# orybkin/video-gcp

Measured on AMD Instinct MI355X. Metric: predicted frames/sec, 64x64x3 seq_len=80 gcp_tree (posterior forward + all loss terms, model(inputs) and model.loss() of train.py:157-159, batch-stat BatchNorm), higher is better.
Workload: dtype f32 (encoder / decoder convs and the tree GEMMs from 512 rows: split-f16 MFMA with f32 accumulate, f32-equivalent; everything else exact f32 MFMA)

## Files before the change

video-gcp_amd/csrc/conv_enc_split.hip:

```cpp
#include "common.h"

#include <cstdlib>

namespace {

typedef _Float16 h8 __attribute__((ext_vector_type(8)));

__device__ __forceinline__ f32x4 mfma32h(h8 a, h8 b, f32x4 c) {
    return __builtin_amdgcn_mfma_f32_16x16x32_f16(a, b, c, 0, 0, 0);
}

template <int CIN, int COUT, int HIN, int FPB, int WP, int WC, bool ZP>
struct EncSplitCfg {
    static constexpr int HOUT = HIN / 2, CT = COUT / 16, CTW = CT / WC;
    static constexpr int PIXB = CIN * 4 + 16;
    static constexpr int NG = FPB * HOUT * HOUT / 16, PGW = (NG + WP - 1) / WP;
    static constexpr int FRAME_PIX = HIN * HIN;
    static constexpr int NSTEP = CIN == 16 ? 8 : 16 * (CIN / 32);
    static constexpr int lds_bytes(int fpb) { return fpb * FRAME_PIX * PIXB + (ZP ? PIXB : 0); }
    static constexpr int LDS_BYTES = lds_bytes(FPB);
    static_assert(WP * WC == 4 && CT % WC == 0 && (HOUT * HOUT) % 16 == 0 && (CIN == 16 || CIN % 32 == 0), "tiling");
};

template <int CIN, int COUT, int HIN, int FPB, int WP, int WC, bool ZP>
__global__ void __launch_bounds__(256) conv4x4s2_split_kernel(const gcpx_conv_args a, const int nblk, const int nrows, const int fpb) {
    using Cfg = EncSplitCfg<CIN, COUT, HIN, FPB, WP, WC, ZP>;
    constexpr int HOUT = Cfg::HOUT, CT = Cfg::CT, CTW = Cfg::CTW, PIXB = Cfg::PIXB, PGW = Cfg::PGW, NSTEP = Cfg::NSTEP;
    constexpr int FRAME_PIX = Cfg::FRAME_PIX, C4 = CIN / 4, C8 = CIN / 8;
    const int tot4 = fpb * FRAME_PIX * C4, tot8 = fpb * FRAME_PIX * C8;
    const int ngrp = fpb * HOUT * HOUT / 16;
    const int npg = __builtin_amdgcn_readfirstlane((ngrp - (int)((threadIdx.x >> 6) % WP) + WP - 1) / WP);
    extern __shared__ float4 encs_smem4[];
    char* lds = reinterpret_cast<char*>(encs_smem4);
    const int tid = threadIdx.x, lane = tid & 63, wave = tid >> 6;
    const int wp = wave % WP, wc = wave / WP;
    const int j = lane & 15, q = lane >> 4;
    const gcpx_conv_src s = a.src[0];
    const int zero_off = fpb * FRAME_PIX * PIXB;
    float* wmax = reinterpret_cast<float*>(lds + CIN * 4);
    if (ZP && tid < PIXB / 4) reinterpret_cast<float*>(lds + zero_off)[tid] = 0.f;
    float4 sc4 = make_float4(1.f, 1.f, 1.f, 1.f), sh4 = make_float4(0.f, 0.f, 0.f, 0.f);
    if (s.scale) {
        sc4 = *reinterpret_cast<const float4*>(s.scale + 4 * (tid % C4));
        sh4 = *reinterpret_cast<const float4*>(s.shift + 4 * (tid % C4));
    }
    const int ew = a.w_split_log2_dev ? __builtin_amdgcn_readfirstlane(*a.w_split_log2_dev) : a.w_split_log2;

    f32x4 st1[CTW], st2[CTW];
#pragma unroll
    for (int ct = 0; ct < CTW; ++ct) { st1[ct] = f32x4{0, 0, 0, 0}; st2[ct] = f32x4{0, 0, 0, 0}; }

    int base[PGW], fl_[PGW], pin_[PGW];
    unsigned vmask[PGW];
#pragma unroll
    for (int pt = 0; pt < PGW; ++pt) {
        const int p = (wp + pt * WP) * 16 + j;
        const int fl = p / (HOUT * HOUT), pin = p % (HOUT * HOUT);
        const int oy = pin / HOUT, ox = pin % HOUT;
        fl_[pt] = fl; pin_[pt] = pin;
        base[pt] = ((fl * HIN + 2 * oy - 1) * HIN + 2 * ox - 1) * PIXB;
        unsigned m = 0;
        for (int k = 0; k < 4; ++k) {
            if (2 * oy - 1 + k >= 0 && 2 * oy - 1 + k < HIN) m |= 1u << k;
            if (2 * ox - 1 + k >= 0 && 2 * ox - 1 + k < HIN) m |= 16u << k;
        }
        vmask[pt] = m;
    }
    const char* wbase = reinterpret_cast<const char*>(a.wpk_split) + (size_t)(wc * CTW) * 2048 + lane * 16;

    for (int blk = blockIdx.x; blk < nblk; blk += gridDim.x) {
        const int f0 = blk * fpb;
        __syncthreads();
        const float4* src = reinterpret_cast<const float4*>(s.ptr) + (size_t)f0 * FRAME_PIX * C4;
        const int nvalid4 = min(fpb, a.F - f0) * FRAME_PIX * C4;
        static_assert(256 % C4 == 0, "staging batches");
        float amax = 0.f;
#pragma unroll 1
        for (int i0 = 0; i0 < tot4; i0 += 256 * 8) {
            float4 v[8];
#pragma unroll
            for (int k = 0; k < 8; ++k) {
                const int idx = i0 + k * 256 + tid;
                v[k] = idx < nvalid4 ? src[idx] : make_float4(0.f, 0.f, 0.f, 0.f);
            }
#pragma unroll
            for (int k = 0; k < 8; ++k) {
                const int idx = i0 + k * 256 + tid;
                const int c4 = idx % C4, pix = idx / C4;
                if (idx < nvalid4) {
                    float4 x = v[k];
                    x.x = fmaf(x.x, sc4.x, sh4.x); x.y = fmaf(x.y, sc4.y, sh4.y); x.z = fmaf(x.z, sc4.z, sh4.z); x.w = fmaf(x.w, sc4.w, sh4.w);
                    if (s.act == GCPX_ACT_LRELU) { x.x = lrelu(x.x, 0.2f); x.y = lrelu(x.y, 0.2f); x.z = lrelu(x.z, 0.2f); x.w = lrelu(x.w, 0.2f); }
                    v[k] = x;
                    amax = fmaxf(amax, fmaxf(fmaxf(fabsf(x.x), fabsf(x.y)), fmaxf(fabsf(x.z), fabsf(x.w))));
                }
                if (idx < tot4) *reinterpret_cast<float4*>(lds + pix * PIXB + 16 * c4) = v[k];
            }
        }
#pragma unroll
        for (int m = 1; m < 64; m <<= 1) amax = fmaxf(amax, __shfl_xor(amax, m));
        if (lane == 0) wmax[wave] = amax;
        __syncthreads();
        amax = fmaxf(fmaxf(wmax[0], wmax[1]), fmaxf(wmax[2], wmax[3]));
        int ex = 14 + 127 - (int)((__float_as_uint(amax) >> 23) & 0xff);
        ex = __builtin_amdgcn_readfirstlane(amax > 0.f ? max(-100, min(min(100, 126 - ew), ex)) : min(100, 126 - ew));
        const float sx2 = __uint_as_float((unsigned)(127 + ex) << 23);
        for (int i = tid; i < tot8; i += 256) {
            const int c8 = i % C8, pix = i / C8;
            char* p = lds + pix * PIXB + 32 * c8;
            const float4 v0 = *reinterpret_cast<const float4*>(p), v1 = *reinterpret_cast<const float4*>(p + 16);
            const float f[8] = {v0.x * sx2, v0.y * sx2, v0.z * sx2, v0.w * sx2, v1.x * sx2, v1.y * sx2, v1.z * sx2, v1.w * sx2};
            h8 p1, p2;
#pragma unroll
            for (int e = 0; e < 8; ++e) {
                p1[e] = (_Float16)f[e];
                p2[e] = (_Float16)fmaf((float)p1[e], -1.f, f[e]);
            }
            *reinterpret_cast<h8*>(p) = p1;
            *reinterpret_cast<h8*>(p + 16) = p2;
        }
        __syncthreads();

        f32x4 acc[CTW][PGW];
#pragma unroll
        for (int ct = 0; ct < CTW; ++ct)
#pragma unroll
            for (int pt = 0; pt < PGW; ++pt) acc[ct][pt] = f32x4{0, 0, 0, 0};
        auto fetch_w = [&](const int step, h8 (&w)[CTW][2]) __attribute__((always_inline)) {
            const char* wp_ = wbase + (size_t)step * CT * 2048;
#pragma unroll
            for (int ct = 0; ct < CTW; ++ct) {
                w[ct][0] = *reinterpret_cast<const h8*>(wp_ + ct * 2048);
                w[ct][1] = *reinterpret_cast<const h8*>(wp_ + ct * 2048 + 1024);
            }
        };
        auto mm = [&](const int step, const h8 (&w)[CTW][2]) __attribute__((always_inline)) {
            const int tap = CIN == 16 ? 2 * step + (q >> 1) : CIN == 32 ? step : step >> 1;
            const int grp = CIN == 16 ? (q & 1) : CIN == 32 ? q : 4 * (step & 1) + q;
            const int ky = tap >> 2, kx = tap & 3;
            const int tapoff = (ky * HIN + kx) * PIXB + grp * 32;
            h8 b[PGW][2];
#pragma unroll
            for (int pt = 0; pt < PGW; ++pt) {
                if (pt >= npg) break;
                const bool ok = ((vmask[pt] >> ky) & 1u) && ((vmask[pt] >> (4 + kx)) & 1u);
                if constexpr (ZP) {
                    const char* p = lds + (ok ? base[pt] + tapoff : zero_off);
                    b[pt][0] = *reinterpret_cast<const h8*>(p);
                    b[pt][1] = *reinterpret_cast<const h8*>(p + 16);
                } else {
                    const char* p = lds + (ok ? base[pt] + tapoff : 0);
                    const h8 t0 = *reinterpret_cast<const h8*>(p), t1 = *reinterpret_cast<const h8*>(p + 16);
                    const h8 z = {0, 0, 0, 0, 0, 0, 0, 0};
                    b[pt][0] = ok ? t0 : z;
                    b[pt][1] = ok ? t1 : z;
                }
            }
#pragma unroll
            for (int ct = 0; ct < CTW; ++ct)
#pragma unroll
                for (int pt = 0; pt < PGW; ++pt) {
                    if (pt >= npg) break;
                    acc[ct][pt] = mfma32h(w[ct][1], b[pt][0], acc[ct][pt]);
                }
#pragma unroll
            for (int ct = 0; ct < CTW; ++ct)
#pragma unroll
                for (int pt = 0; pt < PGW; ++pt) {
                    if (pt >= npg) break;
                    acc[ct][pt] = mfma32h(w[ct][0], b[pt][1], acc[ct][pt]);
                }
#pragma unroll
            for (int ct = 0; ct < CTW; ++ct)
#pragma unroll
                for (int pt = 0; pt < PGW; ++pt) {
                    if (pt >= npg) break;
                    acc[ct][pt] = mfma32h(w[ct][0], b[pt][0], acc[ct][pt]);
                }
        };
        h8 wA[CTW][2], wB[CTW][2];
        static_assert(NSTEP % 2 == 0, "ping-pong");
        fetch_w(0, wA);
#pragma unroll 1
        for (int step = 0; step < NSTEP; step += 2) {
            fetch_w(step + 1, wB);
            mm(step, wA);
            fetch_w(step + 2 < NSTEP ? step + 2 : step, wA);
            mm(step + 1, wB);
        }
        const float inv = __uint_as_float((unsigned)(127 - ex - ew) << 23);
#pragma unroll
        for (int pt = 0; pt < PGW; ++pt) {
            const int f = f0 + fl_[pt];
            if (f >= a.F || wp + pt * WP >= ngrp) continue;
            float* op = a.out + ((size_t)f * HOUT * HOUT + pin_[pt]) * COUT;
#pragma unroll
            for (int ct = 0; ct < CTW; ++ct) {
                const int c = (wc * CTW + ct) * 16 + q * 4;
                const float4 bv = *reinterpret_cast<const float4*>(a.bias + c);
                f32x4 v = acc[ct][pt];
                v[0] = fmaf(v[0], inv, bv.x); v[1] = fmaf(v[1], inv, bv.y); v[2] = fmaf(v[2], inv, bv.z); v[3] = fmaf(v[3], inv, bv.w);
                if (a.out_act == GCPX_ACT_LRELU) {
                    v[0] = lrelu(v[0], 0.2f); v[1] = lrelu(v[1], 0.2f); v[2] = lrelu(v[2], 0.2f); v[3] = lrelu(v[3], 0.2f);
                }
                *reinterpret_cast<float4*>(op + c) = make_float4(v[0], v[1], v[2], v[3]);
                if (a.stats_partial) { st1[ct] += v; st2[ct] += v * v; }
            }
        }
    }
    if (a.stats_partial) {
        __syncthreads();
        float* red = reinterpret_cast<float*>(lds);
#pragma unroll
        for (int ct = 0; ct < CTW; ++ct) {
#pragma unroll
            for (int r = 0; r < 4; ++r) {
                const float s1 = row16_sum(st1[ct][r]);
                const float s2 = row16_sum(st2[ct][r]);
                if (j == 0) {
                    const int c = (wc * CTW + ct) * 16 + q * 4 + r;
                    red[(wp * 2 + 0) * CT * 16 + c] = s1;
                    red[(wp * 2 + 1) * CT * 16 + c] = s2;
                }
            }
        }
        __syncthreads();
        for (int i = tid; i < 2 * CT * 16; i += 256) {
            const int which = i / (CT * 16), c = i % (CT * 16);
            float sum = 0.f;
#pragma unroll
            for (int w_ = 0; w_ < WP; ++w_) sum += red[(w_ * 2 + which) * CT * 16 + c];
            a.stats_partial[((size_t)blockIdx.x * 2 + which) * CT * 16 + c] = sum;
            for (int r = blockIdx.x + gridDim.x; r < nrows; r += gridDim.x) a.stats_partial[((size_t)r * 2 + which) * CT * 16 + c] = 0.f;
        }
    }
}

template <int CIN, int COUT, int HIN, int FPB, int WP, int WC, bool ZP>
int launch_enc_split(const gcpx_conv_args* a, hipStream_t stream, int nrows, int cus) {
    using Cfg = EncSplitCfg<CIN, COUT, HIN, FPB, WP, WC, ZP>;
    auto kern = conv4x4s2_split_kernel<CIN, COUT, HIN, FPB, WP, WC, ZP>;
    static bool attr_set = false;
    if (!attr_set) {
        hipError_t e = hipFuncSetAttribute(reinterpret_cast<const void*>(kern), hipFuncAttributeMaxDynamicSharedMemorySize, Cfg::LDS_BYTES);
        if (e != hipSuccess) {
            gcpx_set_error("conv4x4s2 (split): hipFuncSetAttribute(%d B): %s", Cfg::LDS_BYTES, hipGetErrorString(e));
            return GCPX_ERR_HIP;
        }
        attr_set = true;
    }
    int fpb = 1;
    double best = -1.0;
    const double frame_bytes = 4.0 * (HIN * HIN * CIN + Cfg::HOUT * Cfg::HOUT * COUT);
    const double bank_bytes = 4.0 * 16 * CIN * COUT * (4 / WC) / WP;
    for (int c = 1; c <= FPB; ++c) {
        const int nb = (a->F + c - 1) / c;
        const double cost = (double)((nb + cus - 1) / cus) * (c * frame_bytes + bank_bytes);
        if (best < 0 || cost <= best) { best = cost; fpb = c; }
    }
    if (const char* e = getenv("GCPX_ENC_FPB")) { const int v = atoi(e); if (v >= 1 && v <= FPB) fpb = v; }
    const int nblk = (a->F + fpb - 1) / fpb;
    const int grid = nblk < nrows ? nblk : nrows;
    hipLaunchKernelGGL(kern, dim3(grid), dim3(256), Cfg::lds_bytes(fpb), stream, *a, nblk, nrows, fpb);
    return GCPX_OK;
}

}

int gcpx_launch_enc_split(const gcpx_conv_args* a, hipStream_t stream, int nrows, int cus) {
    if (a->Hin != a->Win) return 1;
    if (a->Cin == 16 && a->Cout == 32 && a->Hin == 32) return launch_enc_split<16, 32, 32, 1, 2, 2, false>(a, stream, nrows, cus);
    if (a->Cin == 32 && a->Cout == 64 && a->Hin == 16) return launch_enc_split<32, 64, 16, 4, 1, 4, true>(a, stream, nrows, cus);
    if (a->Cin == 64 && a->Cout == 128 && a->Hin == 8) return launch_enc_split<64, 128, 8, 8, 1, 4, true>(a, stream, nrows, cus);
    if (a->Cin == 16 && a->Cout == 32 && a->Hin == 16) return launch_enc_split<16, 32, 16, 4, 2, 2, true>(a, stream, nrows, cus);
    if (a->Cin == 32 && a->Cout == 64 && a->Hin == 8) return launch_enc_split<32, 64, 8, 16, 1, 4, true>(a, stream, nrows, cus);
    return 1;
}
```

Measured before the change: 497,000.

## Deepen weight prefetch ring, chunk LDS operand loads, and unmask input staging

```diff
diff --git a/video-gcp_amd/csrc/conv_enc_split.hip b/video-gcp_amd/csrc/conv_enc_split.hip
--- a/video-gcp_amd/csrc/conv_enc_split.hip
+++ b/video-gcp_amd/csrc/conv_enc_split.hip
@@ -17,16 +17,20 @@
     static constexpr int NG = FPB * HOUT * HOUT / 16, PGW = (NG + WP - 1) / WP;
     static constexpr int FRAME_PIX = HIN * HIN;
     static constexpr int NSTEP = CIN == 16 ? 8 : 16 * (CIN / 32);
+    static constexpr int PB = 4;
+    static constexpr int WD = CTW >= 2 ? 3 : 4;
     static constexpr int lds_bytes(int fpb) { return fpb * FRAME_PIX * PIXB + (ZP ? PIXB : 0); }
     static constexpr int LDS_BYTES = lds_bytes(FPB);
     static_assert(WP * WC == 4 && CT % WC == 0 && (HOUT * HOUT) % 16 == 0 && (CIN == 16 || CIN % 32 == 0), "tiling");
 };
 
 template <int CIN, int COUT, int HIN, int FPB, int WP, int WC, bool ZP>
-__global__ void __launch_bounds__(256) conv4x4s2_split_kernel(const gcpx_conv_args a, const int nblk, const int nrows, const int fpb) {
+__global__ void __launch_bounds__(256, 2) conv4x4s2_split_kernel(const gcpx_conv_args a, const int nblk, const int nrows, const int fpb) {
     using Cfg = EncSplitCfg<CIN, COUT, HIN, FPB, WP, WC, ZP>;
     constexpr int HOUT = Cfg::HOUT, CT = Cfg::CT, CTW = Cfg::CTW, PIXB = Cfg::PIXB, PGW = Cfg::PGW, NSTEP = Cfg::NSTEP;
     constexpr int FRAME_PIX = Cfg::FRAME_PIX, C4 = CIN / 4, C8 = CIN / 8;
+    constexpr int PB = Cfg::PB, WD = Cfg::WD, WR = WD + 1;
+    static_assert(WD <= NSTEP, "ring");
     const int tot4 = fpb * FRAME_PIX * C4, tot8 = fpb * FRAME_PIX * C8;
     const int ngrp = fpb * HOUT * HOUT / 16;
     const int npg = __builtin_amdgcn_readfirstlane((ngrp - (int)((threadIdx.x >> 6) % WP) + WP - 1) / WP);
@@ -67,9 +71,20 @@
         vmask[pt] = m;
     }
     const char* wbase = reinterpret_cast<const char*>(a.wpk_split) + (size_t)(wc * CTW) * 2048 + lane * 16;
+    auto fetch_w = [&](const int step, h8 (&w)[CTW][2]) __attribute__((always_inline)) {
+        const char* wp_ = wbase + (size_t)step * CT * 2048;
+#pragma unroll
+        for (int ct = 0; ct < CTW; ++ct) {
+            w[ct][0] = *reinterpret_cast<const h8*>(wp_ + ct * 2048);
+            w[ct][1] = *reinterpret_cast<const h8*>(wp_ + ct * 2048 + 1024);
+        }
+    };
+    h8 wr[WR][CTW][2];
 
     for (int blk = blockIdx.x; blk < nblk; blk += gridDim.x) {
         const int f0 = blk * fpb;
+#pragma unroll
+        for (int d = 0; d < WD; ++d) fetch_w(d, wr[d]);
         __syncthreads();
         const float4* src = reinterpret_cast<const float4*>(s.ptr) + (size_t)f0 * FRAME_PIX * C4;
         const int nvalid4 = min(fpb, a.F - f0) * FRAME_PIX * C4;
@@ -81,19 +96,19 @@
 #pragma unroll
             for (int k = 0; k < 8; ++k) {
                 const int idx = i0 + k * 256 + tid;
-                v[k] = idx < nvalid4 ? src[idx] : make_float4(0.f, 0.f, 0.f, 0.f);
+                v[k] = src[min(idx, nvalid4 - 1)];
             }
 #pragma unroll
             for (int k = 0; k < 8; ++k) {
                 const int idx = i0 + k * 256 + tid;
                 const int c4 = idx % C4, pix = idx / C4;
-                if (idx < nvalid4) {
-                    float4 x = v[k];
-                    x.x = fmaf(x.x, sc4.x, sh4.x); x.y = fmaf(x.y, sc4.y, sh4.y); x.z = fmaf(x.z, sc4.z, sh4.z); x.w = fmaf(x.w, sc4.w, sh4.w);
-                    if (s.act == GCPX_ACT_LRELU) { x.x = lrelu(x.x, 0.2f); x.y = lrelu(x.y, 0.2f); x.z = lrelu(x.z, 0.2f); x.w = lrelu(x.w, 0.2f); }
-                    v[k] = x;
-                    amax = fmaxf(amax, fmaxf(fmaxf(fabsf(x.x), fabsf(x.y)), fmaxf(fabsf(x.z), fabsf(x.w))));
-                }
+                const bool in = idx < nvalid4;
+                float4 x = v[k];
+                x.x = fmaf(x.x, sc4.x, sh4.x); x.y = fmaf(x.y, sc4.y, sh4.y); x.z = fmaf(x.z, sc4.z, sh4.z); x.w = fmaf(x.w, sc4.w, sh4.w);
+                if (s.act == GCPX_ACT_LRELU) { x.x = lrelu(x.x, 0.2f); x.y = lrelu(x.y, 0.2f); x.z = lrelu(x.z, 0.2f); x.w = lrelu(x.w, 0.2f); }
+                const float m = fmaxf(fmaxf(fabsf(x.x), fabsf(x.y)), fmaxf(fabsf(x.z), fabsf(x.w)));
+                amax = fmaxf(amax, in ? m : 0.f);
+                v[k] = in ? x : make_float4(0.f, 0.f, 0.f, 0.f);
                 if (idx < tot4) *reinterpret_cast<float4*>(lds + pix * PIXB + 16 * c4) = v[k];
             }
         }
@@ -126,67 +141,67 @@
         for (int ct = 0; ct < CTW; ++ct)
 #pragma unroll
             for (int pt = 0; pt < PGW; ++pt) acc[ct][pt] = f32x4{0, 0, 0, 0};
-        auto fetch_w = [&](const int step, h8 (&w)[CTW][2]) __attribute__((always_inline)) {
-            const char* wp_ = wbase + (size_t)step * CT * 2048;
-#pragma unroll
-            for (int ct = 0; ct < CTW; ++ct) {
-                w[ct][0] = *reinterpret_cast<const h8*>(wp_ + ct * 2048);
-                w[ct][1] = *reinterpret_cast<const h8*>(wp_ + ct * 2048 + 1024);
-            }
-        };
         auto mm = [&](const int step, const h8 (&w)[CTW][2]) __attribute__((always_inline)) {
             const int tap = CIN == 16 ? 2 * step + (q >> 1) : CIN == 32 ? step : step >> 1;
             const int grp = CIN == 16 ? (q & 1) : CIN == 32 ? q : 4 * (step & 1) + q;
             const int ky = tap >> 2, kx = tap & 3;
             const int tapoff = (ky * HIN + kx) * PIXB + grp * 32;
-            h8 b[PGW][2];
-#pragma unroll
-            for (int pt = 0; pt < PGW; ++pt) {
-                if (pt >= npg) break;
-                const bool ok = ((vmask[pt] >> ky) & 1u) && ((vmask[pt] >> (4 + kx)) & 1u);
-                if constexpr (ZP) {
-                    const char* p = lds + (ok ? base[pt] + tapoff : zero_off);
-                    b[pt][0] = *reinterpret_cast<const h8*>(p);
-                    b[pt][1] = *reinterpret_cast<const h8*>(p + 16);
-                } else {
-                    const char* p = lds + (ok ? base[pt] + tapoff : 0);
-                    const h8 t0 = *reinterpret_cast<const h8*>(p), t1 = *reinterpret_cast<const h8*>(p + 16);
-                    const h8 z = {0, 0, 0, 0, 0, 0, 0, 0};
-                    b[pt][0] = ok ? t0 : z;
-                    b[pt][1] = ok ? t1 : z;
+#pragma unroll
+            for (int p0 = 0; p0 < PGW; p0 += PB) {
+                if (p0 >= npg) break;
+                constexpr int NB = PB < PGW ? PB : PGW;
+                h8 b[NB][2];
+#pragma unroll
+                for (int i = 0; i < NB; ++i) {
+                    const int pt = p0 + i;
+                    if (pt >= PGW || pt >= npg) break;
+                    const bool ok = ((vmask[pt] >> ky) & 1u) && ((vmask[pt] >> (4 + kx)) & 1u);
+                    if constexpr (ZP) {
+                        const char* p = lds + (ok ? base[pt] + tapoff : zero_off);
+                        b[i][0] = *reinterpret_cast<const h8*>(p);
+                        b[i][1] = *reinterpret_cast<const h8*>(p + 16);
+                    } else {
+                        const char* p = lds + (ok ? base[pt] + tapoff : 0);
+                        const h8 t0 = *reinterpret_cast<const h8*>(p), t1 = *reinterpret_cast<const h8*>(p + 16);
+                        const h8 z = {0, 0, 0, 0, 0, 0, 0, 0};
+                        b[i][0] = ok ? t0 : z;
+                        b[i][1] = ok ? t1 : z;
+                    }
                 }
-            }
-#pragma unroll
-            for (int ct = 0; ct < CTW; ++ct)
-#pragma unroll
-                for (int pt = 0; pt < PGW; ++pt) {
-                    if (pt >= npg) break;
-                    acc[ct][pt] = mfma32h(w[ct][1], b[pt][0], acc[ct][pt]);
-                }
-#pragma unroll
-            for (int ct = 0; ct < CTW; ++ct)
-#pragma unroll
-                for (int pt = 0; pt < PGW; ++pt) {
-                    if (pt >= npg) break;
-                    acc[ct][pt] = mfma32h(w[ct][0], b[pt][1], acc[ct][pt]);
-                }
-#pragma unroll
-            for (int ct = 0; ct < CTW; ++ct)
-#pragma unroll
-                for (int pt = 0; pt < PGW; ++pt) {
-                    if (pt >= npg) break;
-                    acc[ct][pt] = mfma32h(w[ct][0], b[pt][0], acc[ct][pt]);
-                }
+#pragma unroll
+                for (int ct = 0; ct < CTW; ++ct)
+#pragma unroll
+                    for (int i = 0; i < NB; ++i) {
+                        const int pt = p0 + i;
+                        if (pt >= PGW || pt >= npg) break;
+                        acc[ct][pt] = mfma32h(w[ct][1], b[i][0], acc[ct][pt]);
+                    }
+#pragma unroll
+                for (int ct = 0; ct < CTW; ++ct)
+#pragma unroll
+                    for (int i = 0; i < NB; ++i) {
+                        const int pt = p0 + i;
+                        if (pt >= PGW || pt >= npg) break;
+                        acc[ct][pt] = mfma32h(w[ct][0], b[i][1], acc[ct][pt]);
+                    }
+#pragma unroll
+                for (int ct = 0; ct < CTW; ++ct)
+#pragma unroll
+                    for (int i = 0; i < NB; ++i) {
+                        const int pt = p0 + i;
+                        if (pt >= PGW || pt >= npg) break;
+                        acc[ct][pt] = mfma32h(w[ct][0], b[i][0], acc[ct][pt]);
+                    }
+            }
         };
-        h8 wA[CTW][2], wB[CTW][2];
-        static_assert(NSTEP % 2 == 0, "ping-pong");
-        fetch_w(0, wA);
 #pragma unroll 1
-        for (int step = 0; step < NSTEP; step += 2) {
-            fetch_w(step + 1, wB);
-            mm(step, wA);
-            fetch_w(step + 2 < NSTEP ? step + 2 : step, wA);
-            mm(step + 1, wB);
+        for (int step = 0; step < NSTEP; step += WR) {
+#pragma unroll
+            for (int r = 0; r < WR; ++r) {
+                if constexpr (NSTEP % WR != 0) { if (step + r >= NSTEP) break; }
+                fetch_w(min(step + r + WD, NSTEP - 1), wr[(r + WD) % WR]);
+                mm(step + r, wr[r]);
+            }
         }
         const float inv = __uint_as_float((unsigned)(127 - ex - ew) << 23);
 #pragma unroll
```

New measurement: 503,100 (median of 6 runs). 1.01x the previous value.
